# voichek/kmersGWAS

Hardware: AMD Instinct MI355X
Metric: k-mers x permutations scored/sec (higher is better)
Workload: dtype fp4 x fp6/fp4 block-scaled filter + f32/f64 exact re-score

## Files before the change

### kmersgwas_amd/csrc/kernels.h

```cpp
#pragma once
#include <hip/hip_runtime.h>
#include <stdint.h>

#include "env.h"
#include "launch.h"

namespace kgwas {

struct Cand {
    uint64_t kmer;
    double score;
    uint64_t row;
};

struct RowSrc {
    const uint32_t* base;
    uint64_t stride_dw;
    uint32_t off_dw;
    uint32_t avail_dw;
};

constexpr uint32_t TESTED_SHARDS = 256;

struct ScoreArgs {
// ... 59 lines not shown
    uint32_t n_kgroups;
    uint32_t n_lgroups;
    uint32_t n_slices;
    const int8_t* Bq;
    const CoarseCol* cols;
    const double* thr;
    unsigned long long* bitmap;
    uint64_t words_per_col;
    unsigned long long* tested;
    float eg_max, rall_max, rmax_max;
};
size_t coarse_lds_bytes(uint32_t n_kgroups, uint32_t T);
hipError_t launch_coarse(const CoarseArgs& a, uint32_t T, uint32_t rows_per_block, hipStream_t st);
struct MxArgs {
    RowSrc src;
    uint64_t n_rows;
    uint32_t S, n_pheno, min_count;
    uint32_t n_full, n_quarter;
    uint32_t n_lgroups;
    uint32_t n_slices;
    uint32_t s1_fp6;
    uint32_t scale0;
    const uint8_t* Bq;
    const CoarseCol* cols;
    const double* thr;
    unsigned long long* bitmap;
    uint64_t words_per_col;
    unsigned long long* tested;
    float eg_max, rall_max, rmax_max;
};
size_t mx_lds_bytes(uint32_t n_steps, uint32_t CT, uint32_t n_slices, uint32_t s1_fp6);
uint32_t mx_step_bytes_rt(uint32_t n_slices, uint32_t s1_fp6);
uint32_t mx_row_tiles(uint32_t CT);
hipError_t launch_mx(const MxArgs& a, uint32_t CT, uint32_t rows_per_block, hipStream_t st);
bool mxs_supported(uint32_t CT, uint32_t NG, uint32_t n_slices, uint32_t s1_fp6);
size_t mxs_lds_bytes(uint32_t CT, uint32_t NG);
hipError_t launch_mxs(const MxArgs& a, uint32_t CT, uint32_t NG, uint32_t form, uint32_t rows_per_block, hipStream_t st);
hipError_t launch_rescore(const ScoreArgs& a, const uint32_t* keys, const uint32_t* surv_off, const uint32_t* surv_cnt,
                          uint32_t row_bits, uint32_t* tile_pref, uint32_t* tile_cnt, double* tmp_score,
                          const uint32_t* key_count, uint32_t* meta, hipStream_t st);
hipError_t launch_rescore_direct(const ScoreArgs& a, const uint32_t* keys, const uint32_t* surv_off, const uint32_t* surv_cnt,
                                 uint32_t row_bits, const uint32_t* tile_pref, hipStream_t st);
struct PrepThr {
    const uint32_t* hist;
    const uint32_t* hist_base;
    uint32_t bins;
    const uint64_t* topn;
    const double* thr_host;
    double* thr;
};
hipError_t launch_chunk_prep(uint32_t* cand_cnt, uint32_t n_pheno, unsigned long long* tested, uint32_t* key_count,
                             unsigned long long* bitmap, uint64_t bitmap_words, uint32_t* seg_cnt, uint32_t n_seg_words, const PrepThr& tu,
                             hipStream_t st);

constexpr int NARROW_SLICES = 3;
constexpr uint32_t NARROW_MAX_COLS = 4;
struct NarrowCol {
    double w[NARROW_SLICES];
    double t1;
    double eg, rall, rmax;
    double pad;
    float wf[3];
    float slackf;
};
struct NarrowArgs {
    RowSrc src;
    uint64_t n_rows;
// ... 127 lines not shown
```

### kmersgwas_amd/csrc/scan_create.cpp

```cpp
#include "scan_internal.h"
#include <chrono>

struct CreateTrace {
    const bool on = opt_set("KGWAS_TRACE");
    const std::chrono::steady_clock::time_point t0 = std::chrono::steady_clock::now();
    void operator()(const char* what) const {
        if (on)
            fprintf(stderr, "[kgwas] scan_create +%.1f ms: %s\n", std::chrono::duration<double, std::milli>(std::chrono::steady_clock::now() - t0).count(), what);
    }
};

static std::unique_ptr<kgwas_scan> new_session(const kgwas_scan_params* p, ScanShape& sh) {
    if (p->struct_size != sizeof(kgwas_scan_params)) throw Error(KGWAS_ERR_ARG, "kgwas_scan_params: size mismatch");
    if (!p->col || !p->Y || !p->topn || p->n_acc == 0 || p->n_pheno == 0 || p->n_acc_file == 0)
        throw Error(KGWAS_ERR_ARG, "kgwas_scan_create: empty problem");
    if (p->n_acc > p->n_acc_file) throw Error(KGWAS_ERR_ARG, "more phenotyped accessions than table columns");
    if (p->n_acc_file >= (1ull << 31)) throw Error(KGWAS_ERR_ARG, "too many accessions");
    require_heap_emulation();
    check_device(p->device);
    KGWAS_HIP(hipSetDevice(p->device));
    std::unique_ptr<kgwas_scan> s(new kgwas_scan);
    s->device = p->device;
    s->S_f = p->n_acc_file;
    s->S = p->n_acc;
    s->W_f = (s->S_f + 63) / 64;
    s->W_m = 2 * ((s->S + 127) / 128);
    s->L = 64 * s->W_m;
    s->n_pheno = p->n_pheno;
    s->min_count = p->min_count;
    s->col.assign(p->col, p->col + s->S);
    s->topn.assign(p->topn, p->topn + s->n_pheno);
    s->Y.assign(p->Y, p->Y + s->n_pheno * s->S);
    if (p->record_history > 2) throw Error(KGWAS_ERR_ARG, "record_history: 0 (off), 1 (full log) or 2 (eviction ring)");
    s->record_history = p->record_history == 1;
    if (p->record_history == 2) {
        s->history_ring = 1;
        if (const char* e = opt_str("KGWAS_HISTORY_RING"))
            if (atoll(e) > 0) s->history_ring = (size_t)atoll(e);
    }
    s->count_patterns = p->count_patterns != 0;
    std::vector<bool> seen(s->S_f, false);
    for (uint64_t i = 0; i < s->S; i++) {
        if (s->col[i] >= s->S_f) throw Error(KGWAS_ERR_ARG, "column index out of range");
        if (seen[s->col[i]]) throw Error(KGWAS_ERR_ARG, "duplicate column index");
        seen[s->col[i]] = true;
    }
    for (uint64_t j = 0; j < s->n_pheno; j++) {
        if (s->topn[j] == 0) throw Error(KGWAS_ERR_ARG, "heap size must be >= 1");
        s->max_topn = std::max(s->max_topn, s->topn[j]);
        s->sum_topn += s->topn[j];
    }
    s->direct = true;
    for (uint64_t i = 0; i < s->S; i++) s->direct = s->direct && (s->col[i] == i);
    if (!s->direct) check_squeeze_fits("kgwas_scan_create", s->S_f, s->S);

// ... 314 lines not shown
```

### kmersgwas_amd/csrc/scan_gpu.cpp

```cpp
#include "scan_internal.h"

namespace kgwas {


void fill_args(kgwas_scan* s, ScoreArgs& a, const uint64_t* d_rows, uint64_t n_rows, uint64_t first_row,
               bool squeezed) {
    memset(&a, 0, sizeof(a));
    if (squeezed) {
        a.src.base = s->d_sq.p;
        a.src.stride_dw = 2 * s->W_m;
        a.src.off_dw = 0;
        a.src.avail_dw = (uint32_t)(2 * s->W_m);
    } else {
        a.src.base = reinterpret_cast<const uint32_t*>(d_rows);
        a.src.stride_dw = 2 * (1 + s->W_f);
        a.src.off_dw = 2;
        a.src.avail_dw = (uint32_t)(2 * s->W_f);
    }
    a.dmask = s->d_dmask.p;
    a.file_rows = d_rows;
    a.file_stride_w = 1 + s->W_f;
    a.n_rows = n_rows;
    a.first_row = first_row;
    a.S = (uint32_t)s->S;
    a.W_m = (uint32_t)s->W_m;
    a.n_pheno = (uint32_t)s->n_pheno;
    a.min_count = (uint32_t)std::min<uint64_t>(s->min_count, 0xFFFFFFFFull);
    a.Yperm = s->d_Yperm.p;
    a.Ymfma = s->d_Ymfma.p;
    a.sums = s->d_sums.p;
    a.thr = s->d_thr.p;
}

uint32_t pick_rows_per_block(uint64_t n_rows, uint64_t ) {
    for (uint32_t rpb : {4096u, 2048u, 1024u, 512u}) {
        if ((n_rows + rpb - 1) / rpb >= 2048) return rpb;
    }
    return 256u;
}

void launch_score(kgwas_scan* s, const ScoreArgs& a) {
    if (s->kernel_used == KGWAS_KERNEL_MFMA) {
        const uint64_t nct = (s->n_pheno + 15) / 16;
        KGWAS_HIP(launch_score_mfma(a, pick_rows_per_block(a.n_rows, nct), s->nb_full, s->stream));
    } else {
        KGWAS_HIP(launch_score_valu(a, s->stream));
    }
    s->st.score_launches++;
}

void maybe_squeeze(kgwas_scan* s, const uint64_t* d_rows, uint64_t n_rows) {
    if (s->direct) return;
    KGWAS_HIP(launch_squeeze(d_rows, 1 + s->W_f, n_rows, s->d_colmap.p, (uint32_t)s->W_m, (uint32_t)s->W_f, s->d_sq.p,
                             s->stream));
}

void hash_patterns(kgwas_scan* s, const uint64_t* d_rows, uint64_t n_rows) {
    const uint64_t need = s->pat_upper + n_rows;
    if (need > s->d_pat.n) {
        DevBuf<uint64_t> bigger;
        bigger.alloc(std::max<uint64_t>(need, 2 * s->d_pat.n));
        if (s->d_pat.n) {
            KGWAS_HIP(hipMemcpyAsync(bigger.p, s->d_pat.p, s->d_pat.n * 8, hipMemcpyDeviceToDevice, s->stream));
            KGWAS_HIP(hipStreamSynchronize(s->stream));
        }
        std::swap(bigger.p, s->d_pat.p);
        std::swap(bigger.n, s->d_pat.n);
    }
    const uint64_t stride = 1 + s->W_f;
    for (uint64_t pos = 0; pos < n_rows; pos += s->chunk_max) {
        const uint64_t c = std::min<uint64_t>(s->chunk_max, n_rows - pos);
        ScoreArgs a;
        fill_args(s, a, d_rows + pos * stride, c, 0, !s->direct);
        maybe_squeeze(s, d_rows + pos * stride, c);
        KGWAS_HIP(launch_pattern_hash(a.src, s->d_dmask.p, c, (uint32_t)s->S, (uint32_t)s->W_m, a.min_count, s->d_pat.p,
                                      s->d_pat_cnt.p, s->stream));
    }
// ... 313 lines not shown
            c.words_per_col = n_words;
            for (uint32_t pi = 0; pi < M.n_parts; pi++) {
                const kgwas_scan::CoarsePart& Pt = M.part[pi];
                c.n_lgroups = Pt.n_lgroups;
                c.Bq = Pt.d_Bq.p;
                c.cols = Pt.d_cols.p;
                c.tested = pi == 0 ? a.tested : nullptr;
                const bool last_part = pi + 1u == M.n_parts;
                const uint32_t rpb = rpb_env ? rpb_env : (n_rows >= (1u << 22) ? 4096u : n_rows >= (1u << 20) ? 2048u : 512u);
                if (M.mx) {
                    MxArgs x;
                    memset(&x, 0, sizeof(x));
                    x.src = c.src;
                    x.n_rows = n_rows;
                    x.S = c.S;
                    x.n_pheno = c.n_pheno;
                    x.min_count = c.min_count;
                    x.n_full = M.mx_full;
                    x.n_quarter = M.mx_quarter;
                    x.n_lgroups = Pt.n_lgroups;
                    x.n_slices = M.slices;
                    x.s1_fp6 = M.mx_s1_fp6;
                    x.scale0 = M.mx_scale0;
                    x.Bq = reinterpret_cast<const uint8_t*>(Pt.d_Bq.p);
                    x.cols = Pt.d_cols.p;
                    x.thr = c.thr;
                    x.bitmap = c.bitmap;
                    x.words_per_col = c.words_per_col;
                    x.tested = c.tested;
                    x.eg_max = c.eg_max;
                    x.rall_max = c.rall_max;
                    x.rmax_max = c.rmax_max;
                    const auto filt = [&] {
                        return Pt.stream ? launch_mxs(x, Pt.T, Pt.ng, Pt.stream - 1u, rpb, s->stream) : launch_mx(x, Pt.T, rpb, s->stream);
                    };
                    if (last_part) KGWAS_HIP(bind_stop(sl.ev_mid, s->stream, filt));
                    else KGWAS_HIP(filt());
                } else {
                    const auto filt = [&] { return launch_coarse(c, Pt.T, rpb, s->stream); };
                    if (last_part) KGWAS_HIP(bind_stop(sl.ev_mid, s->stream, filt));
                    else KGWAS_HIP(filt());
                }
            }
            if (!M.n_parts) KGWAS_HIP(hipEventRecord(sl.ev_mid, s->stream));
        }
        a.tested = nullptr;
        a.so_score = sl.d_so_score.p;
        a.so_kmer = sl.d_so_kmer.p;
        a.so_row = sl.d_so_row.p;
        if (s->narrow) {
            KGWAS_HIP(launch_narrow_keys(s->d_bitmap.p, n_words, n_rows, (uint32_t)s->n_pheno, s->d_bm_blocks.p, s->d_surv_sorted.p, s->key_slots,
                                         s->row_key_bits, s->d_surv_off.p, s->d_surv_cnt.p, s->d_key_count.p, s->d_tile_pref.p, sl.d_meta.p, sl.d_tested.p, s->stream));
            if (s->dbg_keep_surv) dbg_log_survivors(s);
            KGWAS_HIP(bind_stop(sl.ev_k1, s->stream, [&] { return launch_rescore_direct(a, s->d_surv_sorted.p, s->d_surv_off.p, s->d_surv_cnt.p, s->row_key_bits, s->d_tile_pref.p, s->stream); }));
        } else {
        KGWAS_HIP(launch_bitmap_keys(s->d_bitmap.p, n_words, n_rows, (uint32_t)s->n_pheno, s->d_bm_blocks.p, s->d_bm_mask.p, s->d_surv_sorted.p, s->key_slots,
                                     s->row_key_bits, s->d_surv_off.p, s->d_surv_cnt.p, s->d_key_count.p, s->d_tile_pref.p, !s->narrow, s->stream));
        s->bitmap_clean = true;
        if (s->dbg_keep_surv) dbg_log_survivors(s);
        a.so_score = sl.d_so_score.p;
        a.so_kmer = sl.d_so_kmer.p;
        a.so_row = sl.d_so_row.p;
        KGWAS_HIP(bind_stop(sl.ev_k1, s->stream, [&] {
            return launch_rescore(a, s->d_surv_sorted.p, s->d_surv_off.p, s->d_surv_cnt.p, s->row_key_bits, s->d_tile_pref.p,
                                  s->d_tile_cnt.p, s->d_tmp_score.p, s->d_key_count.p, sl.d_meta.p, s->stream);
        }));
        }
// ... 193 lines not shown
```

### kmersgwas_amd/csrc/scan_internal.h

```cpp
#pragma once
#include <algorithm>
#include <atomic>
#include <chrono>
#include <cmath>
#include <condition_variable>
#include <deque>
#include <limits>
#include <cstdio>
#include <cstdlib>
#include <cstring>
#include <functional>
#include <memory>
#include <mutex>
#include <string>
#include <thread>
#include <vector>

#include <dirent.h>
#include <immintrin.h>
#include <pthread.h>
#include <sched.h>
#include <sys/mman.h>

#include "common.h"
// ... 303 lines not shown
    double* so_score = nullptr;
    uint64_t* so_kmer = nullptr;
    uint32_t* so_row = nullptr;
    size_t ring_end = 0;
    DevBuf<double> d_so_score;
    DevBuf<uint64_t> d_so_kmer;
    DevBuf<uint32_t> d_so_row;
    DevBuf<uint32_t> d_meta;
    PinBuf<uint32_t> h_meta;
    uint32_t* h_meta_dev = nullptr;
    double* h_thr_dev = nullptr;
    unsigned long long* h_tested_dev = nullptr;
    PinBuf<double> h_thr;
    bool tie_check = false;
    bool tested_in_meta = false;
    hipEvent_t ev_counts = nullptr;
    DevBuf<unsigned long long> d_tested;
    PinBuf<unsigned long long> h_tested;
    hipEvent_t ev_sq0 = nullptr, ev_k0 = nullptr, ev_k1 = nullptr, ev_done = nullptr, ev_mid = nullptr;
    bool used_coarse = false;
    int coarse_mode = 0;
    double cand_est = 0;
    const uint64_t* rows = nullptr;
    uint64_t first_row = 0, n_rows = 0;
    bool squeezed = false, busy = false;
};

}

using namespace kgwas;

struct kgwas_scan {
    int device = 0;
    uint64_t S_f = 0, S = 0, W_f = 0, W_m = 0, L = 0, n_pheno = 0, min_count = 0;
    std::vector<uint64_t> col, topn;
    std::vector<float> Y;
    bool direct = false;
    uint32_t kernel_used = 0;
    bool record_history = false;
    size_t history_ring = 0;
    uint64_t chunk_max = 0, dense_rows = 0, dense_chunk = 0;
    uint32_t cap = 0;
    uint64_t max_topn = 0;
    uint32_t nb_full = 0;

    hipStream_t stream = nullptr, copy_stream = nullptr;
    hipEvent_t ev_user = nullptr, ev_ds = nullptr, ev_d0 = nullptr, ev_d1 = nullptr;
    hipEvent_t ev_dcopy = nullptr;
    bool dense_copy_pending = false;
    DevBuf<uint32_t> d_dmask, d_colmap, d_sq;
    DevBuf<float> d_Yperm, d_Ymfma, d_sums;
    DevBuf<double> d_thr;
    PinBuf<double> h_thr;
    uint32_t thr_flip = 0;
    DevBuf<uint32_t> d_hist, d_hist_base;
    PinBuf<uint32_t> h_hist_base;
    DevBuf<uint64_t> d_topn;
    DevBuf<double> d_thr_host, d_thr_redo;
    PinBuf<double> h_thr_redo;
    bool hist_ready = false;
    uint64_t rows_submitted = 0;
    bool coarse = false;
    uint32_t n_kgroups = 0;
    struct CoarsePart {
        uint32_t T = 0, n_lgroups = 0;
        uint32_t stream = 0;
// ... 255 lines not shown
```

### kmersgwas_amd/csrc/score_mfma.hip

```cpp
#include "score_common.h"

namespace kgwas {

typedef float f32x4 __attribute__((ext_vector_type(4)));
typedef unsigned int u32x2 __attribute__((ext_vector_type(2)));

#ifndef KGWAS_MFMA_MAX_THREADS
#define KGWAS_MFMA_MAX_THREADS 512
#endif

__device__ __forceinline__ void bcast_rows(uint32_t x, uint32_t (&out)[4]) {
    const u32x2 s = __builtin_amdgcn_permlane32_swap(x, x, false, false);
    const u32x2 a = __builtin_amdgcn_permlane16_swap(s[0], s[0], false, false);
    const u32x2 b = __builtin_amdgcn_permlane16_swap(s[1], s[1], false, false);
    out[0] = a[0];
    out[1] = a[1];
    out[2] = b[0];
    out[3] = b[1];
}

__device__ __forceinline__ uint4 load_piece(const uint32_t* p) {
    const uint2 lo = *reinterpret_cast<const uint2*>(p);
    const uint2 hi = *reinterpret_cast<const uint2*>(p + 2);
    return make_uint4(lo.x, lo.y, hi.x, hi.y);
}

template <int NCT>
__device__ __forceinline__ void mfma_block(f32x4 (&acc)[2][NCT][4], const uint32_t (&w)[2][4], uint32_t sh_e,
                                           uint32_t sh_o, const float* yb, uint32_t ct_stride) {
    float Af[2][4][8];
#pragma unroll
    for (int rt = 0; rt < 2; rt++)
// ... 201 lines not shown
    const uint32_t n_groups = (n_ctiles + NCTMAX - 1) / NCTMAX;
    const uint32_t L = 64u * a.W_m;
    const uint64_t blk_row0 = (uint64_t)rb * rows_per_block;
    for (uint32_t grp = 0; grp < n_groups; grp++) {
        const uint32_t ct0 = grp * NCTMAX;
        const uint32_t nct_here = (n_ctiles - ct0 < (uint32_t)NCTMAX) ? (n_ctiles - ct0) : (uint32_t)NCTMAX;
        if (grp) __syncthreads();
        {
            const float4* src = reinterpret_cast<const float4*>(a.Ymfma + (size_t)ct0 * L * 16u);
            float4* dst = reinterpret_cast<float4*>(ylds);
            for (uint32_t i = threadIdx.x; i < nct_here * L * 4u; i += blockDim.x) dst[i] = src[i];
        }
        __syncthreads();
        if (NCTMAX == 2 && nct_here == 2)
            score_rows<NCTMAX>(a, ylds, ct0, blk_row0, rows_per_block, nb_full);
        else
            score_rows<1>(a, ylds, ct0, blk_row0, rows_per_block, nb_full);
    }
}

size_t mfma_lds_bytes(uint32_t W_m) { return (size_t)64u * W_m * 16u * sizeof(float); }

hipError_t launch_score_mfma(const ScoreArgs& a, uint32_t rows_per_block, uint32_t nb_full, hipStream_t st) {
    if (a.n_rows == 0) return hipSuccess;
    const size_t tile = mfma_lds_bytes(a.W_m);
    if (tile > 160u * 1024u) return hipErrorInvalidValue;
    const uint32_t n_ctiles = (a.n_pheno + 15u) / 16u;
#ifdef KGWAS_PROBE_NCT
    const uint32_t nctmax = KGWAS_PROBE_NCT;
#else
    const uint32_t nctmax = (n_ctiles >= 2 && 2 * tile <= 160u * 1024u) ? 2u : 1u;
#endif
    const size_t lds = tile * nctmax;
    const uint32_t threads = (lds > 80u * 1024u) ? 512u : 256u;
    const uint32_t rpp = (threads >> 6) * 32u;
    rows_per_block = (rows_per_block + rpp - 1) / rpp * rpp;
    const uint32_t n_rowblocks = (uint32_t)((a.n_rows + rows_per_block - 1) / rows_per_block);
    const uint32_t grid = n_rowblocks;
    hipError_t e;
    if (nctmax == 2) {
        if (lds > 64 * 1024 && (e = hipFuncSetAttribute((const void*)score_mfma_kernel<2>,
                                                         hipFuncAttributeMaxDynamicSharedMemorySize, (int)lds)) != hipSuccess)
            return e;
        hipLaunchKernelGGL(score_mfma_kernel<2>, dim3(grid), dim3(threads), lds, st, a, rows_per_block, n_rowblocks,
                           n_ctiles, nb_full);
    } else {
        if (lds > 64 * 1024 && (e = hipFuncSetAttribute((const void*)score_mfma_kernel<1>,
                                                         hipFuncAttributeMaxDynamicSharedMemorySize, (int)lds)) != hipSuccess)
            return e;
        hipLaunchKernelGGL(score_mfma_kernel<1>, dim3(grid), dim3(threads), lds, st, a, rows_per_block, n_rowblocks,
                           n_ctiles, nb_full);
    }
    return hipGetLastError();
}

}
```

### kmersgwas_amd/csrc/score_mx.hip

```cpp
#include <stdlib.h>

#include <algorithm>

#include "score_common.h"

#ifndef KGWAS_MX_ABLATE
#define KGWAS_MX_ABLATE 0
#endif

#ifndef KGWAS_MX_NT
#define KGWAS_MX_NT 0
#endif

#ifndef KGWAS_MX_WARM
#define KGWAS_MX_WARM 0
#endif
#ifndef KGWAS_MX_PERSIST
#define KGWAS_MX_PERSIST 1
#endif

namespace kgwas {

typedef int mxv8i __attribute__((ext_vector_type(8)));
typedef float mxv4f __attribute__((ext_vector_type(4)));

namespace {
constexpr uint32_t MX_PART0 = 1536u;
}

#ifndef KGWAS_MX_PRIO
#define KGWAS_MX_PRIO 0
#endif
#ifndef KGWAS_MX_PRIO_EPI
#define KGWAS_MX_PRIO_EPI 3
#endif
// ... 22 lines not shown
    const uint32_t kb = lane >> 4, m = lane & 15u;
    const uint32_t n_steps = 4u * a.n_full + a.n_quarter;
    const uint32_t group_bytes = n_steps * CT * SB;
    char* lds = reinterpret_cast<char*>(mlds);
    float* colc = reinterpret_cast<float*>(lds + group_bytes);
    const int* colp = reinterpret_cast<const int*>(colc + 2 * SLOTS);
    float* wscr = colc + 3 * SLOTS + wave * (RT * 48u);
    const uint32_t rows_per_pass = (TH / 64) * (RT * 16u);
    const uint64_t blk_row0 = (uint64_t)rb * rows_per_block;
    const float Nf = (float)a.S;
    const char* rows_base = reinterpret_cast<const char*>(a.src.base);
    const uint32_t avail_b = a.src.avail_dw * 4u;
    const int sc0 = (int)a.scale0;
    uint32_t tested_local = 0;

    for (uint32_t lg = lg0; lg < lg1; lg++) {
        if (lg != lg0) __syncthreads();
        {
            const uint4* src = reinterpret_cast<const uint4*>(a.Bq + (size_t)lg * group_bytes);
            for (uint32_t i = threadIdx.x; i < group_bytes / 16u; i += TH) mlds[i] = src[i];
            if (threadIdx.x < SLOTS) {
                const CoarseCol cc = a.cols[lg * SLOTS + threadIdx.x];
                float al = __builtin_huge_valf();
                if (cc.pheno >= 0) al = (float)(sqrt(a.thr[cc.pheno]) * cc.kalpha);
                colc[threadIdx.x] = al;
                colc[SLOTS + threadIdx.x] = cc.iu;
                reinterpret_cast<int*>(colc + 2 * SLOTS)[threadIdx.x] = cc.pheno;
            }
        }
        __syncthreads();

        uint32_t ro[RT];
        const uint64_t wave_row0 = blk_row0 + wave * (RT * 16u);
        auto set_rows = [&](uint32_t (&o)[RT], uint64_t rb0) {
#pragma unroll
            for (int rt = 0; rt < RT; rt++) {
                uint64_t r = rb0 + rt * 16u + m;
                if (r >= a.n_rows) r = a.n_rows - 1;
                o[rt] = ((uint32_t)r * (uint32_t)a.src.stride_dw + a.src.off_dw) * 4u;
            }
        };
        struct __attribute__((aligned(8))) U4 {
            uint32_t x, y, z, w;
        };
        auto load_group = [&](uint32_t (&pc)[RT][4], const uint32_t (&o)[RT], uint32_t g) {
            const uint32_t b0 = 64u * g + 16u * kb;
#pragma unroll
            for (int rt = 0; rt < RT; rt++) {
                uint32_t off = o[rt] + b0;
                asm volatile("" : "+v"(off));
                U4 v;
                if (KGWAS_MX_ABLATE & 8)
                    v = U4{off, lane * 2654435761u, lane, b0};
                else {
#if KGWAS_MX_NT
                    typedef uint32_t nt_u4 __attribute__((ext_vector_type(4), aligned(8)));
                    const nt_u4 t = __builtin_nontemporal_load(reinterpret_cast<const nt_u4*>(rows_base + off));
                    v = U4{t.x, t.y, t.z, t.w};
#else
                    v = *reinterpret_cast<const U4*>(rows_base + off);
#endif
                }
                pc[rt][0] = v.x;
                pc[rt][1] = v.y;
                pc[rt][2] = v.z;
                pc[rt][3] = v.w;
            }
        };
        constexpr int UT = 2;
        constexpr int NU = (CT + UT - 1) / UT;
        typedef uint32_t u32x4 __attribute__((ext_vector_type(4)));
        typedef uint32_t u32x2 __attribute__((ext_vector_type(2)));
// ... 3 lines not shown
        for (int t = 0; t < CT; t++) Bx[t] = Bz[t] = (u32x4){0u, 0u, 0u, 0u}, By[t] = Bv[t] = (u32x2){0u, 0u};
        struct StepAddr {
            uint32_t o16, o8, o8b;
        };
        auto step_addr = [&](const char* bstep) {
            StepAddr sa;
            sa.o16 = (uint32_t)(bstep - lds) + lane * 16u;
            sa.o8 = (uint32_t)(bstep - lds) + lane * 8u + 1024u;
            sa.o8b = sa.o8 + SB;
            asm volatile("" : "+v"(sa.o16), "+v"(sa.o8), "+v"(sa.o8b));
            return sa;
        };
        auto read_unit = [&](int u, const StepAddr& sa) {
#pragma unroll
            for (int t = UT * u; t < (UT * u + UT < CT ? UT * u + UT : CT); t++) {
                if (KGWAS_MX_ABLATE & 4) {
                    Bx[t] = (u32x4){lane, (uint32_t)t, 3u, (uint32_t)u};
                    By[t] = (u32x2){5u, 6u};
                    Bz[t] = (u32x4){lane, (uint32_t)t, 7u, (uint32_t)u};
                    Bv[t] = (u32x2){1u, 2u};
                    continue;
                }
                const char* p16 = lds + sa.o16 + t * SB;
                const char* p8 = (t & 1) ? lds + sa.o8b + (t - 1) * SB : lds + sa.o8 + t * SB;
                Bx[t] = *reinterpret_cast<const u32x4*>(p16);
                By[t] = *reinterpret_cast<const u32x2*>(p8);
                if (NS == 2) {
                    Bz[t] = *reinterpret_cast<const u32x4*>(p16 + MX_PART0);
                    if (S1F == 2) Bv[t] = *reinterpret_cast<const u32x2*>(p8 + MX_PART0);
                }
            }
        };
        uint32_t piece[RT][4];
        const uint64_t pass_stride = persist ? (uint64_t)gridDim.x * rows_per_pass : rows_per_pass;
        const uint64_t wave_row00 = persist ? (uint64_t)blockIdx.x * rows_per_pass + wave * (RT * 16u) : wave_row0;
        const uint64_t n_pass_blk = persist ? ~0ull : (rows_per_block + rows_per_pass - 1) / rows_per_pass;
        set_rows(ro, wave_row00);
        if (a.n_full && wave_row00 < a.n_rows) load_group(piece, ro, 0);
        StepAddr sadr = step_addr(lds);
        read_unit(0, sadr);
        for (uint64_t ps = 0; ps < n_pass_blk; ps++) {
            const uint64_t rbase = wave_row00 + ps * pass_stride;
            if (rbase >= a.n_rows) break;
            uint32_t ro_next[RT];
            set_rows(ro_next, rbase + pass_stride);
#if KGWAS_MX_WARM
            {
                const uint64_t r0 = rbase + pass_stride;
                if (r0 < a.n_rows) {
                    const uint64_t r1 = r0 + RT * 16u < a.n_rows ? r0 + RT * 16u : a.n_rows;
                    const uint32_t b0 = ((uint32_t)r0 * (uint32_t)a.src.stride_dw + a.src.off_dw) * 4u & ~127u;
                    const uint32_t b1 = ((uint32_t)(r1 - 1u) * (uint32_t)a.src.stride_dw + a.src.off_dw) * 4u + avail_b - 4u;
                    asm volatile("s_waitcnt vmcnt(0)" ::: "memory");
                    const uint32_t junk = (uint32_t)(reinterpret_cast<char*>(colc + 3 * SLOTS + (TH / 64) * (RT * 48u)) - lds);
                    const uint32_t n_warm = (b1 - b0) / 8192u + 1u;
                    for (uint32_t k = 0; k < n_warm; k++) {
                        uint32_t off = (b1 - b0) - k * 8192u >= lane * 128u ? b0 + k * 8192u + lane * 128u : b1;
                        asm volatile("s_mov_b32 m0, %0\n\ts_nop 0\n\tglobal_load_lds_dword %1, %2" ::"s"(junk), "v"(off), "s"(rows_base) : "memory");
                    }
                }
            }
#endif
            mxv4f acc[RT][CT];
#pragma unroll
            for (int rt = 0; rt < RT; rt++)
#pragma unroll
                for (int t = 0; t < CT; t++) acc[rt][t] = (mxv4f){0.0f, 0.0f, 0.0f, 0.0f};

            auto mfma_unit = [&](int u, const mxv8i (&A)[RT], int sa) {
#pragma unroll
                for (int t = UT * u; t < (UT * u + UT < CT ? UT * u + UT : CT); t++) {
                    const mxv8i B0 = {(int)Bx[t].x, (int)Bx[t].y, (int)Bx[t].z, (int)Bx[t].w, (int)By[t].x, (int)By[t].y, 0, 0};
#pragma unroll
                    for (int rt = 0; rt < RT; rt++)
                        acc[rt][t] = __builtin_amdgcn_mfma_scale_f32_16x16x128_f8f6f4(A[rt], B0, acc[rt][t], 4, 2, 0, sa, 0, sc0);
                    if (NS == 2) {
                        mxv8i B1 = {(int)Bz[t].x, (int)Bz[t].y, (int)Bz[t].z, (int)Bz[t].w, 0, 0, 0, 0};
                        if (S1F == 2) {
                            B1[4] = (int)Bv[t].x;
                            B1[5] = (int)Bv[t].y;
                        }
#pragma unroll
                        for (int rt = 0; rt < RT; rt++)
                            acc[rt][t] = __builtin_amdgcn_mfma_scale_f32_16x16x128_f8f6f4(A[rt], B1, acc[rt][t], 4, S1F, 0, sa, 0, 0x7F7F7F7F);
                    }
                }
            };
            auto run_step = [&](const mxv8i (&A)[RT], const char* bs_next, int sa) {
                const StepAddr nadr = step_addr(bs_next);
                if (NU == 1) {
                    u32x4 kx[CT], kz[CT];
                    u32x2 ky[CT], kv[CT];
#pragma unroll
                    for (int t = 0; t < CT; t++) kx[t] = Bx[t], ky[t] = By[t], kz[t] = Bz[t], kv[t] = Bv[t];
                    read_unit(0, nadr);
                    u32x4 nx[CT], nz[CT];
                    u32x2 ny[CT], nv[CT];
#pragma unroll
                    for (int t = 0; t < CT; t++) nx[t] = Bx[t], ny[t] = By[t], nz[t] = Bz[t], nv[t] = Bv[t];
#pragma unroll
                    for (int t = 0; t < CT; t++) Bx[t] = kx[t], By[t] = ky[t], Bz[t] = kz[t], Bv[t] = kv[t];
                    __builtin_amdgcn_sched_barrier(0);
                    mfma_unit(0, A, sa);
                    __builtin_amdgcn_sched_barrier(0);
#pragma unroll
                    for (int t = 0; t < CT; t++) Bx[t] = nx[t], By[t] = ny[t], Bz[t] = nz[t], Bv[t] = nv[t];
                } else {
#pragma unroll
                    for (int u = 0; u < NU; u++) {
                        if (u + 1 < NU)
                            read_unit(u + 1, sadr);
                        else
                            read_unit(0, nadr);
                        __builtin_amdgcn_sched_barrier(0);
                        mfma_unit(u, A, sa);
                        __builtin_amdgcn_sched_barrier(0);
                    }
                }
                sadr = nadr;
            };

#if KGWAS_MX_PRIO || KGWAS_MX_PRIO_EPI
            __builtin_amdgcn_s_setprio(KGWAS_MX_PRIO);
#endif
            for (uint32_t g = 0; g < a.n_full; g++) {
                const char* bg = lds + (size_t)g * 4u * CT * SB;
                const bool last_g = g + 1u == a.n_full;
#pragma unroll
                for (int j = 0; j < 4; j++) {
                    mxv8i A[RT];
#pragma unroll
                    for (int rt = 0; rt < RT; rt++) {
                        A[rt] = (mxv8i){0, 0, 0, 0, 0, 0, 0, 0};
#pragma unroll
                        for (int q = 0; q < 4; q++) {
                            if (KGWAS_MX_ABLATE & 2)
                                A[rt][q] = (int)piece[rt][q];
                            else
                                A[rt][q] = j < 3 ? (int)(piece[rt][q] & (0x11111111u << j)) : (int)((piece[rt][q] >> 1) & 0x44444444u);
                        }
                    }
                    const char* bs = bg + j * CT * SB;
                    const char* bs_next = bs + CT * SB;
                    if (j == 3) {
                        __builtin_amdgcn_sched_barrier(0);
                        uint32_t on[RT];
#pragma unroll
                        for (int rt = 0; rt < RT; rt++) on[rt] = last_g ? ro_next[rt] : ro[rt];
                        load_group(piece, on, last_g ? 0u : g + 1u);
                        if (last_g && a.n_quarter == 0) bs_next = lds;
                        __builtin_amdgcn_sched_barrier(0);
                    }
                    run_step(A, bs_next, j == 0 ? 0x7F7F7F7F : j == 1 ? 0x7E7E7E7E : 0x7D7D7D7D);
                }
            }
            for (uint32_t x = 0; x < a.n_quarter; x++) {
                uint32_t b0 = 64u * a.n_full + 16u * x + 4u * kb;
                b0 = b0 + 4u <= avail_b ? b0 : avail_b - 4u;
                mxv8i A[RT];
#pragma unroll
                for (int rt = 0; rt < RT; rt++) {
                    const uint32_t w = (KGWAS_MX_ABLATE & 8) ? ro[rt] + b0 : *reinterpret_cast<const uint32_t*>(rows_base + (ro[rt] + b0));
                    A[rt] = (mxv8i){(int)(w & 0x11111111u), (int)((w >> 1) & 0x11111111u), (int)((w >> 2) & 0x11111111u),
                                    (int)((w >> 3) & 0x11111111u), 0, 0, 0, 0};
                }
                const char* bs = lds + (size_t)(4u * a.n_full + x) * CT * SB;
                run_step(A, x + 1u == a.n_quarter ? lds : bs + CT * SB, 0x7F7F7F7F);
            }

#if KGWAS_MX_PRIO || KGWAS_MX_PRIO_EPI
            __builtin_amdgcn_s_setprio(KGWAS_MX_PRIO_EPI);
#endif
            float2* trm = reinterpret_cast<float2*>(wscr + RT * 16);
            {
                float* n1s = wscr;
                if (m == 15u) {
#pragma unroll
                    for (int rt = 0; rt < RT; rt++) *reinterpret_cast<mxv4f*>(n1s + kb * (RT * 4u) + rt * 4) = acc[rt][CT - 1];
                }
                __builtin_amdgcn_wave_barrier();
                const uint64_t left = a.n_rows - rbase;
                const uint32_t rows_here = left < RT * 16u ? (uint32_t)left : RT * 16u;
                const bool mac_any = a.S >= 2u * a.min_count;
                const uint32_t span = a.S - 2u * a.min_count;
#pragma unroll
                for (int w = 0; w < NW; w++) {
                    const uint32_t e = lane + 64u * w;
                    const uint32_t kbe = e / (RT * 4u), ie = e % (RT * 4u);
                    const uint32_t row = 16u * (ie >> 2) + 4u * kbe + (ie & 3u);
                    const float f = n1s[e];
                    const uint32_t n1r = (uint32_t)f;
                    const bool ok = mac_any & (row < rows_here) & ((n1r - a.min_count) <= span);
                    if (lg == 0) tested_local += ok ? 1u : 0u;
                    const float sq = __builtin_amdgcn_sqrtf(f * (Nf - f)) * 0.99999905f;
                    float2 tm;
                    tm.x = ok ? sq : __builtin_huge_valf();
                    tm.y = (a.eg_max + fminf(a.rall_max, f * a.rmax_max)) * 1.000001f;
                    trm[e] = tm;
                }
                __builtin_amdgcn_wave_barrier();
            }

            float alc[CT];
            float al_min = __builtin_huge_valf();
#pragma unroll
            for (int t = 0; t < CT; t++) {
                alc[t] = colc[t * 16 + m];
                al_min = fminf(al_min, alc[t]);
            }
            const bool ones_lane = m == 15u;
#pragma unroll
            for (int w = 0; w < NW; w++) {
                float sqd[16], er[16];
#pragma unroll
                for (int i = 0; i < 16; i += 2) {
// ... 16 lines not shown
                        const float v = acc[gi >> 2][CT - 1][gi & 3];
                        mx[i] = ones_lane ? 0.0f : fabsf(v);
                    }
#pragma unroll
                    for (int t = 0; t + 1 < CT; t++)
#pragma unroll
                        for (int i = 0; i < 16; i++) {
                            const int gi = 16 * w + i;
                            mx[i] = fmaxf(mx[i], fabsf(acc[gi >> 2][t][gi & 3]));
                        }
#pragma unroll
                    for (int i = 0; i < 16; i++) hit[i] = __ballot(fmaf(-al_min, sqd[i], mx[i]) + er[i] >= 0.0f);
                } else {
#pragma unroll
                    for (int i = 0; i < 16; i++) hit[i] = 0;
                    int x = 0;
#pragma unroll
                    for (int i = 0; i < 16; i++)
#pragma unroll
                        for (int t = 0; t < CT; t++) x ^= __float_as_int(acc[(16 * w + i) >> 2][t][i & 3]);
                    hit[0] = __ballot(x == 0x7fffffff);
                }
                uint64_t hit_any = 0;
#pragma unroll
                for (int i = 0; i < 16; i++) hit_any |= hit[i];
                if ((KGWAS_MX_ABLATE & 32) && hit_any) {
                    if (lane == 0) atomicAdd(&a.tested[0], 0ull);
                    hit_any = 0;
                }
                if (hit_any) {
                    uint32_t mb[CT];
#pragma unroll
                    for (int t = 0; t < CT; t++) mb[t] = 0;
#pragma unroll
                    for (int i = 0; i < 16; i++) {
                        if (hit[i]) {
#pragma unroll
                            for (int t = 0; t < CT; t++) {
                                float al = alc[t];
                                asm volatile("" : "+v"(al));
                                mb[t] |= (pair_margin(i, t, al) + er[i] >= 0.0f) ? (1u << i) : 0u;
                            }
                        }
                    }
                    unsigned short* bm16 = reinterpret_cast<unsigned short*>(a.bitmap) + ((rbase >> 6) + w) * 4u + kb;
#pragma unroll
                    for (int t = 0; t < CT; t++)
                        if (mb[t]) bm16[(uint64_t)colp[t * 16 + m] * a.words_per_col * 4u] = (unsigned short)mb[t];
                }
            }
            __builtin_amdgcn_wave_barrier();
#pragma unroll
            for (int rt = 0; rt < RT; rt++) ro[rt] = ro_next[rt];
        }
    }
#if KGWAS_MX_WARM
    asm volatile("s_waitcnt vmcnt(0)" ::: "memory");
#endif
    if (a.tested) {
        uint32_t v = tested_local;
#pragma unroll
        for (int d = 1; d < 64; d <<= 1) v += __shfl_xor(v, d);
        if (lane == 0u && v) atomicAdd(&a.tested[blockIdx.x % TESTED_SHARDS], (unsigned long long)v);
    }
}

size_t mx_lds_bytes(uint32_t n_steps, uint32_t CT, uint32_t n_slices, uint32_t s1_fp6) {
    const uint32_t sb = n_slices == 1 ? MX_PART0 : (s1_fp6 ? 2u * MX_PART0 : MX_PART0 + 1024u);
    return (size_t)n_steps * CT * sb + 3u * 112u * 4u + 12u * 768u + 256u;
}
uint32_t mx_step_bytes_rt(uint32_t n_slices, uint32_t s1_fp6) { return n_slices == 1 ? MX_PART0 : (s1_fp6 ? 2u * MX_PART0 : MX_PART0 + 1024u); }
uint32_t mx_row_tiles(uint32_t CT) { return 4u; }

template <int CT, int RT, int NS, int S1F, int TH = 512>
static hipError_t launch_mx_t(const MxArgs& a, uint32_t rows_per_block, size_t lds, hipStream_t st) {
    const uint32_t rpp = (TH / 64) * RT * 16u;
    rows_per_block = (rows_per_block + rpp - 1) / rpp * rpp;
    const uint32_t n_rowblocks = (uint32_t)((a.n_rows + rows_per_block - 1) / rows_per_block);
    if (lds > 64 * 1024) {
        hipError_t e = hipFuncSetAttribute((const void*)mx_kernel<CT, RT, NS, S1F, TH>, hipFuncAttributeMaxDynamicSharedMemorySize, (int)lds);
        if (e != hipSuccess) return e;
    }
    const uint32_t grid_lg = a.n_lgroups > 1 ? 1u : 0u;
    uint32_t grid = grid_lg ? (n_rowblocks + 7u) / 8u * 8u * a.n_lgroups : n_rowblocks;
    if (KGWAS_MX_PERSIST && !grid_lg) {
        static int n_cu = 0;
        if (!n_cu) {
            int dev = 0;
            hipDeviceProp_t pr;
            n_cu = (hipGetDevice(&dev) == hipSuccess && hipGetDeviceProperties(&pr, dev) == hipSuccess && pr.multiProcessorCount > 0) ? pr.multiProcessorCount : 256;
        }
        const uint64_t n_pass = (a.n_rows + rpp - 1) / rpp;
        grid = (uint32_t)std::min<uint64_t>(n_pass, (uint64_t)n_cu);
    }
    launch_last(mx_kernel<CT, RT, NS, S1F, TH>, dim3(grid), dim3(TH), lds, st, a, rows_per_block, n_rowblocks, grid_lg);
    return hipGetLastError();
}

template <int NS, int S1F>
static hipError_t launch_mx_ct(const MxArgs& a, uint32_t CT, uint32_t rows_per_block, size_t lds, hipStream_t st) {
    switch (CT) {
        case 1: return launch_mx_t<1, 4, NS, S1F, 768>(a, rows_per_block, lds, st);
        case 2: return launch_mx_t<2, 4, NS, S1F, 768>(a, rows_per_block, lds, st);
        case 3: return launch_mx_t<3, 4, NS, S1F, 768>(a, rows_per_block, lds, st);
        case 4: return launch_mx_t<4, 4, NS, S1F>(a, rows_per_block, lds, st);
        case 5: return launch_mx_t<5, 4, NS, S1F>(a, rows_per_block, lds, st);
        case 6: return launch_mx_t<6, 4, NS, S1F>(a, rows_per_block, lds, st);
        case 7: return launch_mx_t<7, 4, NS, S1F>(a, rows_per_block, lds, st);
    }
    return hipErrorInvalidValue;
}

hipError_t launch_mx(const MxArgs& a, uint32_t CT, uint32_t rows_per_block, hipStream_t st) {
    if (a.n_rows == 0) return hipSuccess;
    const size_t lds = mx_lds_bytes(4u * a.n_full + a.n_quarter, CT, a.n_slices, a.s1_fp6);
    if (lds > 160u * 1024u) return hipErrorInvalidValue;
    if ((a.n_rows * a.src.stride_dw + a.src.off_dw + a.src.avail_dw) * 4ull >= (1ull << 32)) return hipErrorInvalidValue;
#ifdef KGWAS_MX_BENCH_ONLY
    if (a.n_slices == 2 && !a.s1_fp6 && CT == 7) return launch_mx_t<7, 4, 2, 4>(a, rows_per_block, lds, st);
    return hipErrorInvalidValue;
#else
    if (a.n_slices == 1) return launch_mx_ct<1, 4>(a, CT, rows_per_block, lds, st);
    if (a.n_slices == 2 && !a.s1_fp6) return launch_mx_ct<2, 4>(a, CT, rows_per_block, lds, st);
    if (a.n_slices == 2 && a.s1_fp6) return launch_mx_ct<2, 2>(a, CT, rows_per_block, lds, st);
    return hipErrorInvalidValue;
#endif
}

}
```

Before: 541.8 billion.

## Trim MX kernel register use and adapt block sizing to CU count

After: 542.9 billion (median of 2 runs). About the same (+0.2%).

```diff
diff --git a/kmersgwas_amd/csrc/kernels.h b/kmersgwas_amd/csrc/kernels.h
--- a/kmersgwas_amd/csrc/kernels.h
+++ b/kmersgwas_amd/csrc/kernels.h
@@ -115,7 +115,7 @@
 size_t mx_lds_bytes(uint32_t n_steps, uint32_t CT, uint32_t n_slices, uint32_t s1_fp6);
 uint32_t mx_step_bytes_rt(uint32_t n_slices, uint32_t s1_fp6);
 uint32_t mx_row_tiles(uint32_t CT);
-hipError_t launch_mx(const MxArgs& a, uint32_t CT, uint32_t rows_per_block, hipStream_t st);
+hipError_t launch_mx(const MxArgs& a, uint32_t CT, uint32_t rows_per_block, uint32_t n_cu, hipStream_t st);
 bool mxs_supported(uint32_t CT, uint32_t NG, uint32_t n_slices, uint32_t s1_fp6);
 size_t mxs_lds_bytes(uint32_t CT, uint32_t NG);
 hipError_t launch_mxs(const MxArgs& a, uint32_t CT, uint32_t NG, uint32_t form, uint32_t rows_per_block, hipStream_t st);
diff --git a/kmersgwas_amd/csrc/scan_create.cpp b/kmersgwas_amd/csrc/scan_create.cpp
--- a/kmersgwas_amd/csrc/scan_create.cpp
+++ b/kmersgwas_amd/csrc/scan_create.cpp
@@ -21,6 +21,11 @@
     KGWAS_HIP(hipSetDevice(p->device));
     std::unique_ptr<kgwas_scan> s(new kgwas_scan);
     s->device = p->device;
+    {
+        int n_cu = 0;
+        KGWAS_HIP(hipDeviceGetAttribute(&n_cu, hipDeviceAttributeMultiprocessorCount, p->device));
+        if (n_cu > 0) s->n_cu = (uint32_t)n_cu;
+    }
     s->S_f = p->n_acc_file;
     s->S = p->n_acc;
     s->W_f = (s->S_f + 63) / 64;
diff --git a/kmersgwas_amd/csrc/scan_gpu.cpp b/kmersgwas_amd/csrc/scan_gpu.cpp
--- a/kmersgwas_amd/csrc/scan_gpu.cpp
+++ b/kmersgwas_amd/csrc/scan_gpu.cpp
@@ -32,17 +32,17 @@
     a.thr = s->d_thr.p;
 }
 
-uint32_t pick_rows_per_block(uint64_t n_rows, uint64_t ) {
+uint32_t pick_rows_per_block(uint64_t n_rows, uint32_t n_cu) {
     for (uint32_t rpb : {4096u, 2048u, 1024u, 512u}) {
         if ((n_rows + rpb - 1) / rpb >= 2048) return rpb;
     }
+    if ((n_rows + 255u) / 256u < n_cu) return 128u;
     return 256u;
 }
 
 void launch_score(kgwas_scan* s, const ScoreArgs& a) {
     if (s->kernel_used == KGWAS_KERNEL_MFMA) {
-        const uint64_t nct = (s->n_pheno + 15) / 16;
-        KGWAS_HIP(launch_score_mfma(a, pick_rows_per_block(a.n_rows, nct), s->nb_full, s->stream));
+        KGWAS_HIP(launch_score_mfma(a, pick_rows_per_block(a.n_rows, s->n_cu), s->nb_full, s->stream));
     } else {
         KGWAS_HIP(launch_score_valu(a, s->stream));
     }
@@ -422,7 +422,7 @@
                     x.rall_max = c.rall_max;
                     x.rmax_max = c.rmax_max;
                     const auto filt = [&] {
-                        return Pt.stream ? launch_mxs(x, Pt.T, Pt.ng, Pt.stream - 1u, rpb, s->stream) : launch_mx(x, Pt.T, rpb, s->stream);
+                        return Pt.stream ? launch_mxs(x, Pt.T, Pt.ng, Pt.stream - 1u, rpb, s->stream) : launch_mx(x, Pt.T, rpb, s->n_cu, s->stream);
                     };
                     if (last_part) KGWAS_HIP(bind_stop(sl.ev_mid, s->stream, filt));
                     else KGWAS_HIP(filt());
diff --git a/kmersgwas_amd/csrc/scan_internal.h b/kmersgwas_amd/csrc/scan_internal.h
--- a/kmersgwas_amd/csrc/scan_internal.h
+++ b/kmersgwas_amd/csrc/scan_internal.h
@@ -359,6 +359,7 @@
 
 struct kgwas_scan {
     int device = 0;
+    uint32_t n_cu = 256;
     uint64_t S_f = 0, S = 0, W_f = 0, W_m = 0, L = 0, n_pheno = 0, min_count = 0;
     std::vector<uint64_t> col, topn;
     std::vector<float> Y;
diff --git a/kmersgwas_amd/csrc/score_mfma.hip b/kmersgwas_amd/csrc/score_mfma.hip
--- a/kmersgwas_amd/csrc/score_mfma.hip
+++ b/kmersgwas_amd/csrc/score_mfma.hip
@@ -1,3 +1,5 @@
+#include <algorithm>
+
 #include "score_common.h"
 
 namespace kgwas {
@@ -265,7 +267,7 @@
     const uint32_t nctmax = (n_ctiles >= 2 && 2 * tile <= 160u * 1024u) ? 2u : 1u;
 #endif
     const size_t lds = tile * nctmax;
-    const uint32_t threads = (lds > 80u * 1024u) ? 512u : 256u;
+    const uint32_t threads = std::min((lds > 80u * 1024u) ? 512u : 256u, std::max(1u, (rows_per_block + 31u) / 32u) * 64u);
     const uint32_t rpp = (threads >> 6) * 32u;
     rows_per_block = (rows_per_block + rpp - 1) / rpp * rpp;
     const uint32_t n_rowblocks = (uint32_t)((a.n_rows + rows_per_block - 1) / rows_per_block);
diff --git a/kmersgwas_amd/csrc/score_mx.hip b/kmersgwas_amd/csrc/score_mx.hip
--- a/kmersgwas_amd/csrc/score_mx.hip
+++ b/kmersgwas_amd/csrc/score_mx.hip
@@ -1,6 +1,7 @@
 #include <stdlib.h>
 
 #include <algorithm>
+#include <type_traits>
 
 #include "score_common.h"
 
@@ -89,12 +90,13 @@
 
         uint32_t ro[RT];
         const uint64_t wave_row0 = blk_row0 + wave * (RT * 16u);
-        auto set_rows = [&](uint32_t (&o)[RT], uint64_t rb0) {
+        auto set_rows = [&](uint32_t (&o)[RT], uint32_t rb0) {
+            uint32_t mm = m;
+            asm volatile("" : "+v"(mm));
 #pragma unroll
             for (int rt = 0; rt < RT; rt++) {
-                uint64_t r = rb0 + rt * 16u + m;
-                if (r >= a.n_rows) r = a.n_rows - 1;
-                o[rt] = ((uint32_t)r * (uint32_t)a.src.stride_dw + a.src.off_dw) * 4u;
+                const uint32_t r = std::min(rb0 + rt * 16u + mm, (uint32_t)a.n_rows - 1u);
+                o[rt] = (r * (uint32_t)a.src.stride_dw + a.src.off_dw) * 4u;
             }
         };
         struct __attribute__((aligned(8))) U4 {
@@ -164,21 +166,23 @@
             }
         };
         uint32_t piece[RT][4];
-        const uint64_t pass_stride = persist ? (uint64_t)gridDim.x * rows_per_pass : rows_per_pass;
-        const uint64_t wave_row00 = persist ? (uint64_t)blockIdx.x * rows_per_pass + wave * (RT * 16u) : wave_row0;
-        const uint64_t n_pass_blk = persist ? ~0ull : (rows_per_block + rows_per_pass - 1) / rows_per_pass;
+        const uint32_t n_rows32 = (uint32_t)a.n_rows;
+        const uint32_t pass_stride = persist ? gridDim.x * rows_per_pass : rows_per_pass;
+        const uint32_t wave_row00 = persist ? blockIdx.x * rows_per_pass + wave * (RT * 16u) : (uint32_t)wave_row0;
+        const uint32_t n_pass_blk = persist ? ~0u : (rows_per_block + rows_per_pass - 1) / rows_per_pass;
+        const uint32_t ro_step = pass_stride * (uint32_t)a.src.stride_dw * 4u;
         set_rows(ro, wave_row00);
-        if (a.n_full && wave_row00 < a.n_rows) load_group(piece, ro, 0);
+        if (a.n_full && wave_row00 < n_rows32) load_group(piece, ro, 0);
         StepAddr sadr = step_addr(lds);
         read_unit(0, sadr);
-        for (uint64_t ps = 0; ps < n_pass_blk; ps++) {
-            const uint64_t rbase = wave_row00 + ps * pass_stride;
-            if (rbase >= a.n_rows) break;
-            uint32_t ro_next[RT];
-            set_rows(ro_next, rbase + pass_stride);
+        for (uint32_t ps = 0; ps < n_pass_blk; ps++) {
+            const uint32_t rbase = wave_row00 + ps * pass_stride;
+            if (rbase >= n_rows32) break;
+            const bool next_whole = rbase + pass_stride + RT * 16u <= n_rows32;
+            const uint32_t ro_adv = next_whole ? ro_step : 0u;
 #if KGWAS_MX_WARM
             {
-                const uint64_t r0 = rbase + pass_stride;
+                const uint64_t r0 = (uint64_t)rbase + pass_stride;
                 if (r0 < a.n_rows) {
                     const uint64_t r1 = r0 + RT * 16u < a.n_rows ? r0 + RT * 16u : a.n_rows;
                     const uint32_t b0 = ((uint32_t)r0 * (uint32_t)a.src.stride_dw + a.src.off_dw) * 4u & ~127u;
@@ -194,18 +198,19 @@
             }
 #endif
             mxv4f acc[RT][CT];
-#pragma unroll
-            for (int rt = 0; rt < RT; rt++)
-#pragma unroll
-                for (int t = 0; t < CT; t++) acc[rt][t] = (mxv4f){0.0f, 0.0f, 0.0f, 0.0f};
-
-            auto mfma_unit = [&](int u, const mxv8i (&A)[RT], int sa) {
+
+            auto mfma_unit = [&](auto first, int u, const mxv8i (&A)[RT], int sa) {
+                constexpr bool FIRST = decltype(first)::value;
 #pragma unroll
                 for (int t = UT * u; t < (UT * u + UT < CT ? UT * u + UT : CT); t++) {
                     const mxv8i B0 = {(int)Bx[t].x, (int)Bx[t].y, (int)Bx[t].z, (int)Bx[t].w, (int)By[t].x, (int)By[t].y, 0, 0};
 #pragma unroll
-                    for (int rt = 0; rt < RT; rt++)
-                        acc[rt][t] = __builtin_amdgcn_mfma_scale_f32_16x16x128_f8f6f4(A[rt], B0, acc[rt][t], 4, 2, 0, sa, 0, sc0);
+                    for (int rt = 0; rt < RT; rt++) {
+                        if (FIRST)
+                            acc[rt][t] = __builtin_amdgcn_mfma_scale_f32_16x16x128_f8f6f4(A[rt], B0, (mxv4f){0.0f, 0.0f, 0.0f, 0.0f}, 4, 2, 0, sa, 0, sc0);
+                        else
+                            acc[rt][t] = __builtin_amdgcn_mfma_scale_f32_16x16x128_f8f6f4(A[rt], B0, acc[rt][t], 4, 2, 0, sa, 0, sc0);
+                    }
                     if (NS == 2) {
                         mxv8i B1 = {(int)Bz[t].x, (int)Bz[t].y, (int)Bz[t].z, (int)Bz[t].w, 0, 0, 0, 0};
                         if (S1F == 2) {
@@ -218,7 +223,7 @@
                     }
                 }
             };
-            auto run_step = [&](const mxv8i (&A)[RT], const char* bs_next, int sa) {
+            auto run_step = [&](auto first, const mxv8i (&A)[RT], const char* bs_next, int sa) {
                 const StepAddr nadr = step_addr(bs_next);
                 if (NU == 1) {
                     u32x4 kx[CT], kz[CT];
@@ -233,7 +238,7 @@
 #pragma unroll
                     for (int t = 0; t < CT; t++) Bx[t] = kx[t], By[t] = ky[t], Bz[t] = kz[t], Bv[t] = kv[t];
                     __builtin_amdgcn_sched_barrier(0);
-                    mfma_unit(0, A, sa);
+                    mfma_unit(first, 0, A, sa);
                     __builtin_amdgcn_sched_barrier(0);
 #pragma unroll
                     for (int t = 0; t < CT; t++) Bx[t] = nx[t], By[t] = ny[t], Bz[t] = nz[t], Bv[t] = nv[t];
@@ -245,7 +250,7 @@
                         else
                             read_unit(0, nadr);
                         __builtin_amdgcn_sched_barrier(0);
-                        mfma_unit(u, A, sa);
+                        mfma_unit(first, u, A, sa);
                         __builtin_amdgcn_sched_barrier(0);
                     }
                 }
@@ -255,7 +260,8 @@
 #if KGWAS_MX_PRIO || KGWAS_MX_PRIO_EPI
             __builtin_amdgcn_s_setprio(KGWAS_MX_PRIO);
 #endif
-            for (uint32_t g = 0; g < a.n_full; g++) {
+            auto full_group = [&](auto first, uint32_t g) __attribute__((always_inline)) {
+                asm volatile("" : "+s"(g));
                 const char* bg = lds + (size_t)g * 4u * CT * SB;
                 const bool last_g = g + 1u == a.n_full;
 #pragma unroll
@@ -278,15 +284,20 @@
                         __builtin_amdgcn_sched_barrier(0);
                         uint32_t on[RT];
 #pragma unroll
-                        for (int rt = 0; rt < RT; rt++) on[rt] = last_g ? ro_next[rt] : ro[rt];
+                        for (int rt = 0; rt < RT; rt++) on[rt] = ro[rt] + (last_g ? ro_adv : 0u);
                         load_group(piece, on, last_g ? 0u : g + 1u);
                         if (last_g && a.n_quarter == 0) bs_next = lds;
                         __builtin_amdgcn_sched_barrier(0);
                     }
-                    run_step(A, bs_next, j == 0 ? 0x7F7F7F7F : j == 1 ? 0x7E7E7E7E : 0x7D7D7D7D);
-                }
-            }
-            for (uint32_t x = 0; x < a.n_quarter; x++) {
+                    const int sa = j == 0 ? 0x7F7F7F7F : j == 1 ? 0x7E7E7E7E : 0x7D7D7D7D;
+                    if (decltype(first)::value && j == 0)
+                        run_step(std::true_type(), A, bs_next, sa);
+                    else
+                        run_step(std::false_type(), A, bs_next, sa);
+                }
+            };
+            auto quarter_step = [&](auto first, uint32_t x) __attribute__((always_inline)) {
+                asm volatile("" : "+s"(x));
                 uint32_t b0 = 64u * a.n_full + 16u * x + 4u * kb;
                 b0 = b0 + 4u <= avail_b ? b0 : avail_b - 4u;
                 mxv8i A[RT];
@@ -297,8 +308,13 @@
                                     (int)((w >> 3) & 0x11111111u), 0, 0, 0, 0};
                 }
                 const char* bs = lds + (size_t)(4u * a.n_full + x) * CT * SB;
-                run_step(A, x + 1u == a.n_quarter ? lds : bs + CT * SB, 0x7F7F7F7F);
-            }
+                run_step(first, A, x + 1u == a.n_quarter ? lds : bs + CT * SB, 0x7F7F7F7F);
+            };
+            uint32_t xq = 0;
+            if (a.n_full) full_group(std::true_type(), 0u);
+            for (uint32_t g = 1; g < a.n_full; g++) full_group(std::false_type(), g);
+            if (!a.n_full) quarter_step(std::true_type(), xq++);
+            for (; xq < a.n_quarter; xq++) quarter_step(std::false_type(), xq);
 
 #if KGWAS_MX_PRIO || KGWAS_MX_PRIO_EPI
             __builtin_amdgcn_s_setprio(KGWAS_MX_PRIO_EPI);
@@ -311,8 +327,8 @@
                     for (int rt = 0; rt < RT; rt++) *reinterpret_cast<mxv4f*>(n1s + kb * (RT * 4u) + rt * 4) = acc[rt][CT - 1];
                 }
                 __builtin_amdgcn_wave_barrier();
-                const uint64_t left = a.n_rows - rbase;
-                const uint32_t rows_here = left < RT * 16u ? (uint32_t)left : RT * 16u;
+                const uint32_t left = n_rows32 - rbase;
+                const uint32_t rows_here = left < RT * 16u ? left : RT * 16u;
                 const bool mac_any = a.S >= 2u * a.min_count;
                 const uint32_t span = a.S - 2u * a.min_count;
 #pragma unroll
@@ -395,6 +411,8 @@
                     uint32_t mb[CT];
 #pragma unroll
                     for (int t = 0; t < CT; t++) mb[t] = 0;
+                    uint32_t one = 1u;
+                    asm volatile("" : "+v"(one));
 #pragma unroll
                     for (int i = 0; i < 16; i++) {
                         if (hit[i]) {
@@ -402,7 +420,7 @@
                             for (int t = 0; t < CT; t++) {
                                 float al = alc[t];
                                 asm volatile("" : "+v"(al));
-                                mb[t] |= (pair_margin(i, t, al) + er[i] >= 0.0f) ? (1u << i) : 0u;
+                                mb[t] |= (pair_margin(i, t, al) + er[i] >= 0.0f) ? (one << i) : 0u;
                             }
                         }
                     }
@@ -413,8 +431,13 @@
                 }
             }
             __builtin_amdgcn_wave_barrier();
-#pragma unroll
-            for (int rt = 0; rt < RT; rt++) ro[rt] = ro_next[rt];
+            if (next_whole) {
+#pragma unroll
+                for (int rt = 0; rt < RT; rt++) ro[rt] += ro_step;
+            } else {
+                set_rows(ro, rbase + pass_stride);
+                if (a.n_full && rbase + pass_stride < n_rows32) load_group(piece, ro, 0);
+            }
         }
     }
 #if KGWAS_MX_WARM
@@ -436,7 +459,7 @@
 uint32_t mx_row_tiles(uint32_t CT) { return 4u; }
 
 template <int CT, int RT, int NS, int S1F, int TH = 512>
-static hipError_t launch_mx_t(const MxArgs& a, uint32_t rows_per_block, size_t lds, hipStream_t st) {
+static hipError_t launch_mx_t(const MxArgs& a, uint32_t rows_per_block, uint32_t n_cu, size_t lds, hipStream_t st) {
     const uint32_t rpp = (TH / 64) * RT * 16u;
     rows_per_block = (rows_per_block + rpp - 1) / rpp * rpp;
     const uint32_t n_rowblocks = (uint32_t)((a.n_rows + rows_per_block - 1) / rows_per_block);
@@ -447,12 +470,6 @@
     const uint32_t grid_lg = a.n_lgroups > 1 ? 1u : 0u;
     uint32_t grid = grid_lg ? (n_rowblocks + 7u) / 8u * 8u * a.n_lgroups : n_rowblocks;
     if (KGWAS_MX_PERSIST && !grid_lg) {
-        static int n_cu = 0;
-        if (!n_cu) {
-            int dev = 0;
-            hipDeviceProp_t pr;
-            n_cu = (hipGetDevice(&dev) == hipSuccess && hipGetDeviceProperties(&pr, dev) == hipSuccess && pr.multiProcessorCount > 0) ? pr.multiProcessorCount : 256;
-        }
         const uint64_t n_pass = (a.n_rows + rpp - 1) / rpp;
         grid = (uint32_t)std::min<uint64_t>(n_pass, (uint64_t)n_cu);
     }
@@ -461,31 +478,32 @@
 }
 
 template <int NS, int S1F>
-static hipError_t launch_mx_ct(const MxArgs& a, uint32_t CT, uint32_t rows_per_block, size_t lds, hipStream_t st) {
+static hipError_t launch_mx_ct(const MxArgs& a, uint32_t CT, uint32_t rows_per_block, uint32_t n_cu, size_t lds, hipStream_t st) {
     switch (CT) {
-        case 1: return launch_mx_t<1, 4, NS, S1F, 768>(a, rows_per_block, lds, st);
-        case 2: return launch_mx_t<2, 4, NS, S1F, 768>(a, rows_per_block, lds, st);
-        case 3: return launch_mx_t<3, 4, NS, S1F, 768>(a, rows_per_block, lds, st);
-        case 4: return launch_mx_t<4, 4, NS, S1F>(a, rows_per_block, lds, st);
-        case 5: return launch_mx_t<5, 4, NS, S1F>(a, rows_per_block, lds, st);
-        case 6: return launch_mx_t<6, 4, NS, S1F>(a, rows_per_block, lds, st);
-        case 7: return launch_mx_t<7, 4, NS, S1F>(a, rows_per_block, lds, st);
+        case 1: return launch_mx_t<1, 4, NS, S1F, 768>(a, rows_per_block, n_cu, lds, st);
+        case 2: return launch_mx_t<2, 4, NS, S1F, 768>(a, rows_per_block, n_cu, lds, st);
+        case 3: return launch_mx_t<3, 4, NS, S1F, 768>(a, rows_per_block, n_cu, lds, st);
+        case 4: return launch_mx_t<4, 4, NS, S1F>(a, rows_per_block, n_cu, lds, st);
+        case 5: return launch_mx_t<5, 4, NS, S1F>(a, rows_per_block, n_cu, lds, st);
+        case 6: return launch_mx_t<6, 4, NS, S1F>(a, rows_per_block, n_cu, lds, st);
+        case 7: return launch_mx_t<7, 4, NS, S1F>(a, rows_per_block, n_cu, lds, st);
     }
     return hipErrorInvalidValue;
 }
 
-hipError_t launch_mx(const MxArgs& a, uint32_t CT, uint32_t rows_per_block, hipStream_t st) {
+hipError_t launch_mx(const MxArgs& a, uint32_t CT, uint32_t rows_per_block, uint32_t n_cu, hipStream_t st) {
     if (a.n_rows == 0) return hipSuccess;
+    if (4u * a.n_full + a.n_quarter == 0u || n_cu == 0u) return hipErrorInvalidValue;
     const size_t lds = mx_lds_bytes(4u * a.n_full + a.n_quarter, CT, a.n_slices, a.s1_fp6);
     if (lds > 160u * 1024u) return hipErrorInvalidValue;
     if ((a.n_rows * a.src.stride_dw + a.src.off_dw + a.src.avail_dw) * 4ull >= (1ull << 32)) return hipErrorInvalidValue;
 #ifdef KGWAS_MX_BENCH_ONLY
-    if (a.n_slices == 2 && !a.s1_fp6 && CT == 7) return launch_mx_t<7, 4, 2, 4>(a, rows_per_block, lds, st);
+    if (a.n_slices == 2 && !a.s1_fp6 && CT == 7) return launch_mx_t<7, 4, 2, 4>(a, rows_per_block, n_cu, lds, st);
     return hipErrorInvalidValue;
 #else
-    if (a.n_slices == 1) return launch_mx_ct<1, 4>(a, CT, rows_per_block, lds, st);
-    if (a.n_slices == 2 && !a.s1_fp6) return launch_mx_ct<2, 4>(a, CT, rows_per_block, lds, st);
-    if (a.n_slices == 2 && a.s1_fp6) return launch_mx_ct<2, 2>(a, CT, rows_per_block, lds, st);
+    if (a.n_slices == 1) return launch_mx_ct<1, 4>(a, CT, rows_per_block, n_cu, lds, st);
+    if (a.n_slices == 2 && !a.s1_fp6) return launch_mx_ct<2, 4>(a, CT, rows_per_block, n_cu, lds, st);
+    if (a.n_slices == 2 && a.s1_fp6) return launch_mx_ct<2, 2>(a, CT, rows_per_block, n_cu, lds, st);
     return hipErrorInvalidValue;
 #endif
 }
```
